# tier4/icp_rust

Measured on AMD Instinct MI355X. Metric: ICP iterations/sec on 1M-pt 3D pair, higher is better.
Workload: dtype f64

## Files before the change

### icp_rust_amd/_lib.py

```python
import ctypes as C
import os
import subprocess

_HERE = os.path.dirname(os.path.abspath(__file__))
_CSRC = os.path.join(_HERE, "csrc")
LIB_PATH = os.environ.get("ICP_MI355X_LIB") or os.path.join(_HERE, "lib", "libicp_mi355x.so")

OK, NONE, EMPTY_DST, NAN_INPUT, BAD_ARGUMENT, NO_DEVICE, HIP_ERROR, OUT_OF_MEMORY, RETRY_REPLICATED, RETRY_SHARDED = range(10)
NN_AUTO, NN_BRUTE, NN_GRID = 0, 1, 2


class Pose(C.Structure):

    _fields_ = [(n, C.c_double) for n in ("r00", "r10", "r01", "r11", "tx", "ty")]

    def as_tuple(self):
        return (self.r00, self.r10, self.r01, self.r11, self.tx, self.ty)


class BatchItem(C.Structure):

    _fields_ = [("src_first", C.c_uint64), ("n", C.c_uint64), ("dst_first", C.c_uint64), ("m", C.c_uint64),
                ("init", Pose)]

# ... 94 lines not shown
    "icp_estimate_transform_device": (C.c_int, [_vp, _vp, _vp, _sz, _pp, _vp]),
    "icp_nn_search_device": (C.c_int, [_vp, _vp, _sz, _vp]),
    "icp_weighted_gn_step_device": (C.c_int, [_vp, _vp, _vp, _sz, _pp, C.c_int, _dp, _dp]),
    "icp_shard_geometry": (C.c_int, [_sz, C.c_int, C.c_int, C.POINTER(C.c_int), C.POINTER(C.c_int),
                                     C.POINTER(C.c_int), C.POINTER(_sz)]),
    "icp_shard_histogram_words": (_sz, []),
    "icp_shard_candidates_bytes": (_sz, []),
    "icp_shard_partials_bytes": (_sz, [C.c_int]),
    "icp_shard_exchange_bytes": (_sz, [C.c_int]),
    "icp_shard_take_device": (C.c_int, [_vp, _vp, _vp, _sz, C.c_int, C.c_int, _sz]),
    "icp_shard_put_device": (C.c_int, [_vp, _vp, _vp, _sz, C.c_int, C.c_int, _sz]),
    "icp_shard_eval_hist_device": (C.c_int, [_vp, _vp, _vp, _sz, C.c_int, C.c_int, _pp, C.c_int, C.c_int,
                                             C.POINTER(_vp)]),
    "icp_shard_eval_compact_device": (C.c_int, [_vp, _vp]),
    "icp_shard_eval_finish_device": (C.c_int, [_vp, _vp, _dp, _dp]),
    "icp_create_multi": (C.c_int, [C.POINTER(_vp), C.c_int, _vp, _sz, C.POINTER(C.c_int), C.c_int]),
    "icp_multi_estimate": (C.c_int, [_vp, _vp, _sz, _pp, _sz, _pp, _vp, _vp]),
    "icp_multi_counters": (C.c_int, [_vp, C.POINTER(C.c_uint64)]),
    "icp_multi_loop_counters": (C.c_int, [_vp, C.POINTER(C.c_uint64)]),
    "icp_multi_pipe_iterations": (C.c_int, [_vp, C.POINTER(C.c_uint64)]),
    "icp_pipe_counters": (C.c_int, [_vp, C.POINTER(C.c_uint64)]),
    "icp_debug_sort_cells": (C.c_int, [_vp, _sz, C.c_uint, _vp, _vp]),
    "icp_set_fixed_point_exit": (C.c_int, [_vp, C.c_int]),
    "icp_shard_pipe_run_device": (C.c_int, [_vp, _vp, _sz, _sz, C.c_int, C.c_int, _pp, C.POINTER(_sz), _sz, _vp, _vp,
                                            C.POINTER(C.c_int)]),
    "icp_loop_inbox_bytes": (_sz, []),
    "icp_loop_inbox": (C.c_int, [_vp, C.c_int, C.POINTER(C.c_void_p)]),
    "icp_loop_inbox_ipc_handle": (C.c_int, [_vp, C.c_char_p]),
    "icp_loop_ipc_open": (C.c_int, [C.c_int, C.c_char_p, C.POINTER(C.c_void_p)]),
    "icp_loop_ipc_close": (C.c_int, [_vp]),
    "icp_loop_inbox_shm_name": (C.c_int, [_vp, C.c_char_p]),
    "icp_loop_inbox_shm_unlink": (C.c_int, [_vp]),
    "icp_loop_shm_open": (C.c_int, [C.c_int, C.c_char_p, C.POINTER(C.c_void_p)]),
    "icp_loop_shm_close": (C.c_int, [_vp]),
    "icp_loop_transport_probe": (C.c_int, [_vp, C.c_int, C.POINTER(C.c_int)]),
    "icp_reset_window_predictions": (C.c_int, [_vp]),
    "icp_shard_loop_connect": (C.c_int, [_vp, C.c_int, C.c_int, C.POINTER(C.c_void_p)]),
    "icp_shard_loop_launch_device": (C.c_int, [_vp, _vp, _vp, _sz, C.c_uint, C.c_uint, C.c_int, C.c_uint32, _pp, C.c_double,
                                               C.c_int, C.c_int]),
    "icp_shard_loop_wait": (C.c_int, [_vp, _pp, C.POINTER(C.c_double), _u32p, C.POINTER(C.c_int), C.POINTER(C.c_int), _u32p]),
    "icp_destroy_multi": (None, [_vp]),
    "icp_synchronize": (C.c_int, [_vp]),
    "icp_profile_enable": (C.c_int, [_vp, C.c_int]),
    "icp_profile_read": (C.c_int, [_vp, _dp, C.POINTER(C.c_uint64)]),
    "icp_reduce_geometry": (None, [_sz, C.POINTER(C.c_int), C.POINTER(C.c_int)]),
    "icp_nn_cert_counters": (C.c_int, [_vp, C.POINTER(C.c_uint64)]),
# ... 154 lines not shown
```

### icp_rust_amd/csrc/api.hip

```cpp
#include <dlfcn.h>
#include <fcntl.h>
#include <sys/mman.h>
#include <unistd.h>

#include <cfloat>
#include <chrono>
#include <cstdio>
#include <cstring>
#include <atomic>
#include <map>
#include <mutex>
#include <new>

#include "api_internal.hpp"

using namespace icp;
using namespace icp::api;

namespace icp {
namespace api {
int map_hip(hipError_t e) {
  switch (e) {
    case hipSuccess: return ICP_OK;
    case hipErrorOutOfMemory: return ICP_OUT_OF_MEMORY;
// ... 332 lines not shown
void free_handle(icp_handle *h) {
  (void)hipSetDevice(h->device);
  free_workspace(h->ws);
  (void)hipFree(h->d_dst_own);
  (void)hipFree(h->d_dst_soa);
  (void)hipFree(h->d_dst_f32);
  (void)hipFree(h->grid.d_start);
  (void)hipFree(h->grid.d_pts);
  (void)hipFree(h->grid.t_cell_of);
  (void)hipFree(h->grid.t_cnt);
  (void)hipFree(h->grid.t_btot);
  (void)hipFree(h->grid.t_part);
  (void)hipFree(h->grid.d_rcell);
  (void)hipFree(h->grid.d_rcell2);
  (void)hipFree(h->grid.d_start2);
  (void)hipFree(h->grid.d_pts2);
  (void)hipFree(h->grid.t_shift);
  (void)hipFree(h->grid.t_cell_new);
  (void)hipFree(h->grid.d_flag);
  (void)hipFree(h->qsort.d_cell_of);
  (void)hipFree(h->qsort.d_tmp);
  (void)hipFree(h->qsort.d_cert_lists);
  (void)hipFree(h->qsort.d_cert_ctr);
  (void)hipFree(h->qsort.d_perm);
  (void)hipFree(h->qsort.d_sorted);
  (void)hipFree(h->qsort.d_prev);
  (void)hipFree(h->shard.d_ordered);
  (void)hipFree(h->d_normals);
  (void)hipFree(h->d_dst_alt);
  (void)hipFree(h->d_normals_alt);
  (void)hipFree(h->d_plane_pairs);
  (void)hipFree(h->d_plane_fa);
  (void)hipFree(h->d_plane_fb);
  (void)hipFree(h->d_plane_stage);
  if (h->own_stream) (void)hipStreamDestroy(h->own_stream);
  delete h;
}

constexpr size_t kPoolMax = 2;
std::mutex g_pool_mu;
std::vector<icp_handle *> g_pool;

}

static void destroy_failed(icp_handle *h) {
  (void)hipSetDevice(h->device);
// ... 15 lines not shown

extern "C" void icp_destroy(icp_handle *h) {
  if (!h) return;
  (void)hipSetDevice(h->device);
  if (h->own_stream) (void)hipStreamSynchronize(h->own_stream);
  if (h->stream != h->own_stream) (void)hipStreamSynchronize(h->stream);
  if (h->ws.spec_stream) (void)hipStreamSynchronize(h->ws.spec_stream);
  for (auto *v : {&h->prof_events, &h->prof_free}) {
    for (auto &ev : *v) {
      (void)hipEventDestroy(ev.first);
      (void)hipEventDestroy(ev.second);
    }
    v->clear();
  }
  static const bool no_pool = getenv("ICP_NO_POOL") != nullptr;
  if (!no_pool) {
    Workspace &w = h->ws;
    h->m = 0;
    h->d_dst = nullptr;
    h->owns_dst = false;
    h->nn_mode = ICP_NN_AUTO;
    h->single_launch = true;
    h->fixed_point_exit = true;
    h->stream = h->own_stream;
    h->profile = 0;
    h->prof_seen = 0;
    h->grid.built = false;
    h->grid.appends_moved = h->grid.appends_rebuilt = 0;
    h->grid.crops_moved = h->grid.crops_rebuilt = 0;
    h->grid.thins_moved = h->grid.thins_rebuilt = 0;
    h->grid.filters_moved = h->grid.filters_rebuilt = 0;
    h->grid.removes_moved = h->grid.removes_rebuilt = 0;
    h->grid.queries_cell = h->grid.queries_caller = 0;
    h->grid.query_force = 0;
    h->qsort.valid = false;
    h->qsort.have_prev = false;
    h->qsort.slot_order = false;
    h->qsort.fold_n = 0;
    h->qsort.last_cert_ctr = nullptr;
    h->qsort.cert_searches = 0;
    h->qsort.have_certs = false;
    h->shard.active = false;
    h->shard.refined_ready = h->shard.attempt_refined = false;
    h->normals_m = 0;
    h->normals_k = 0;
    for (int k = 0; k < 5; ++k) {
// ... 45 lines not shown
static constexpr long kGridMinM = 8192;

int icp::api::resolved_nn_mode(const icp_handle *h) {
  if (h->nn_mode == ICP_NN_BRUTE || !h->grid.built) return ICP_NN_BRUTE;
  if (h->nn_mode == ICP_NN_GRID) return ICP_NN_GRID;
  return (long)h->m >= kGridMinM ? ICP_NN_GRID : ICP_NN_BRUTE;
}

static hipError_t launch_nn(icp_handle *h, const double *d_src, size_t n, const Pose *T, double *d_a,
                            double *d_b, uint32_t *d_idx) {
  Range range("icp: search (transform + exact nearest neighbour + pairs)");
  if (resolved_nn_mode(h) == ICP_NN_GRID) return launch_nn_grid(h, d_src, n, T, d_a, d_b, d_idx);
  return launch_nn_brute(h, d_src, n, T, d_a, d_b, d_idx);
}

extern "C" int icp_set_single_launch(icp_handle *h, int enable) {
  if (!h) return ICP_BAD_ARGUMENT;
  h->single_launch = enable != 0;
  return ICP_OK;
}
extern "C" int icp_set_fixed_point_exit(icp_handle *h, int enable) {
  if (!h) return ICP_BAD_ARGUMENT;
  h->fixed_point_exit = enable != 0;
  return ICP_OK;
}
extern "C" int icp_single_launch_counters(icp_handle *h, uint64_t out[3]) {
  if (!h || !out) return ICP_BAD_ARGUMENT;
  out[0] = h->ws.tiny_calls;
  out[1] = h->ws.tiny_evals;
  out[2] = h->ws.tiny_sorted;
  return ICP_OK;
}
extern "C" int icp_get_nn_mode(const icp_handle *h) {
  if (!h) return ICP_BAD_ARGUMENT;
  return resolved_nn_mode(h);
}
extern "C" int icp_set_stream(icp_handle *h, void *s) {
  if (!h) return ICP_BAD_ARGUMENT;
  h->stream = (hipStream_t)s;
  return ICP_OK;
}
extern "C" int icp_use_own_stream(icp_handle *h) {
  if (!h) return ICP_BAD_ARGUMENT;
  h->stream = h->own_stream;
  return ICP_OK;
}
// ... 880 lines not shown
```

### icp_rust_amd/csrc/common.hpp

```cpp
#pragma once
#include <hip/hip_runtime.h>

#include <cstddef>
#include <cstdint>
#include <cstdlib>
#include <utility>
#include <vector>

#include "pose.hpp"

namespace icp {


struct Range {
  explicit Range(const char *name);
  ~Range();
  Range(const Range &) = delete;
  Range &operator=(const Range &) = delete;
};

constexpr int kReduceThreads = 512;
constexpr int kReduceMaxBlocks = 256;
constexpr int kTreeMaxBlocks = 2048;
constexpr int kShardMaxWorld = 16;
// ... 257 lines not shown
struct QuerySort {
  bool valid = false;
  bool slot_order = false;
  bool identity = false;
  bool presorted = false;
  bool sort_only = false;
  size_t fold_n = 0;
  const double *src = nullptr;
  size_t n = 0, cap = 0;
  uint32_t *d_cell_of = nullptr;
  uint32_t *d_perm = nullptr;
  void *d_tmp = nullptr;
  size_t cap_tmp = 0;
  bool have_prev = false;
  PrevMatch *d_prev = nullptr;
  double *d_sorted = nullptr;
  bool have_certs = false, have_pose = false, have_pose_before = false;
  double decay_r = 0., decay_t = 0.;
  Pose last_pose;
  uint32_t *d_cert_lists = nullptr;
  unsigned *d_cert_ctr = nullptr, *last_cert_ctr = nullptr;
  unsigned cert_seq = 0;
  unsigned long long cert_searches = 0;
};

hipError_t stable_sort_cells(const uint32_t *keys_in, uint32_t *perm_out, unsigned n, unsigned bits, void *&tmp, size_t &cap_tmp,
                             hipStream_t s);

}

struct icp_handle {
  int dim = 0;
  size_t m = 0;
  int device = 0;
  int nn_mode = ICP_NN_AUTO;
  bool single_launch = true;
  bool fixed_point_exit = true;
  bool owns_dst = false;
  const double *d_dst = nullptr;
  double *d_dst_own = nullptr;
  size_t cap_dst_own = 0, cap_soa = 0, cap_f32 = 0;
  double *d_dst_soa = nullptr;
  float *d_dst_f32 = nullptr;
  size_t m_pad = 0;
  bool brute_valid = false;
  bool screen_valid = false;
  hipStream_t own_stream = nullptr;
  hipStream_t stream = nullptr;
  icp::Workspace ws;
  icp::Grid grid;
  icp::QuerySort qsort;
  struct ShardEval {
    icp::WinParams P;
    int kind = 2, rank = 0, world = 1, b0 = 0, b1 = 0, blocks = 0;
    size_t n_local = 0, n_total = 0;
    const double *d_a = nullptr;
    icp::Pose T;
    double *d_ordered = nullptr;
    bool active = false;
    icp::WinParams P2;
// ... 211 lines not shown
```

### icp_rust_amd/csrc/nn_grid.hip

```cpp
#include "common.hpp"
#include <type_traits>

namespace icp {

__device__ __forceinline__ int cell_coord(double v, double lo, double inv_h, int n) {
  double t = floor((v - lo) * inv_h);
  t = fmin(fmax(t, 0.), (double)(n - 1));
  return (int)t;
}

__global__ void k_grid_bbox(const double *__restrict__ dst, unsigned m, int dim, double *__restrict__ part) {
  __shared__ double smn[3][256], smx[3][256];
  double mn[3], mx[3];
  for (int d = 0; d < 3; ++d) {
    mn[d] = __builtin_huge_val();
    mx[d] = -__builtin_huge_val();
  }
  for (unsigned i = blockIdx.x * 256 + threadIdx.x; i < m; i += gridDim.x * 256)
    for (int d = 0; d < dim; ++d) {
      const double v = dst[(size_t)i * dim + d];
      mn[d] = fmin(mn[d], v);
      mx[d] = fmax(mx[d], v);
    }
  for (int d = 0; d < 3; ++d) {
// ... 929 lines not shown
                                                               GridParams g, const uint32_t *__restrict__ start,
                                                               const GridPoint *__restrict__ pts,
                                                               const double *__restrict__ dst, uint32_t *__restrict__ idx,
                                                               double2 *__restrict__ a, double2 *__restrict__ b,
                                                               PrevMatch *prev, CertDecay cd, unsigned xcd_chunk) {
  const unsigned k = xcd_wave(blockIdx.x, gridDim.x, xcd_chunk) * kGridThreads + threadIdx.x;
  if (k >= n) return;
  warm_query<DIM, CERT>(k, src, perm, T, g, start, pts, dst, idx, a, b, prev, cd);
}

#ifndef ICP_COOP_ITEMS
#define ICP_COOP_ITEMS 2
#endif
#ifndef ICP_COOP_ROWS
#define ICP_COOP_ROWS 4
#endif
#ifndef ICP_COOP_FLUSH_AT
#define ICP_COOP_FLUSH_AT 96
#endif
constexpr int kCoopItems = ICP_COOP_ITEMS;
constexpr int kCoopRows = ICP_COOP_ROWS;
constexpr int kCoopCandCap = 256;
constexpr int kCoopFlushAt = ICP_COOP_FLUSH_AT;
struct CoopLds {
  uint32_t pref[64];
  uint32_t rows_d[64][kCoopRows];
  uint32_t rows_o[64][kCoopRows];
  float4 oq[64];
  uint32_t obi[64];
  uint2 cand[kCoopCandCap];
  unsigned long long fkey[64];
  uint32_t fidx[64];
  uint32_t fwin[64];
};

#ifdef ICP_COOP_PROFILE
__device__ unsigned long long g_coop_prof[64][12];
__device__ long long g_coop_span[16384][2];
__device__ unsigned long long g_coop_rows[32];
#define COOP_STAMP(i)                                                  \
  do {                                                                 \
    asm volatile("s_waitcnt vmcnt(0) lgkmcnt(0)" ::: "memory");        \
    const long long now_ = wall_clock64();                             \
    cprof[i] += (unsigned long long)(now_ - ct_last);                  \
    ct_last = now_;                                                    \
  } while (0)
#define COOP_COUNT(i, v) (cprof[i] += (v))
#else
#define COOP_STAMP(i) ((void)0)
#define COOP_COUNT(i, v) ((void)0)
#endif

template <int DIM, bool SEEDED>
__device__ __forceinline__ void warm_wave(const unsigned k, const unsigned n, const double *__restrict__ src,
                                          const uint32_t *__restrict__ perm, Pose T, const GridParams &g,
                                          const uint32_t *__restrict__ start, const GridPoint *__restrict__ pts,
                                          const double *__restrict__ dst, uint32_t *__restrict__ idx,
                                          double2 *__restrict__ a, double2 *__restrict__ b, PrevMatch *prev, PrevMatch seed,
                                          CoopLds &S) {
  const unsigned lane = threadIdx.x;
#ifdef ICP_COOP_PROFILE
  unsigned long long cprof[12] = {0, 0, 0, 0, 0, 0, 0, 1, 0, 0, 0, 0};
  long long ct_last = wall_clock64();
  const long long ct_first = ct_last;
#endif
  const bool in_range = k < n;
  const unsigned kk = in_range ? k : n - 1;
  const unsigned i = perm ? perm[kk] : kk;
  double q[3];
  q[0] = src[(size_t)kk * DIM + 0];
  q[1] = src[(size_t)kk * DIM + 1];
  q[2] = DIM == 3 ? src[(size_t)kk * DIM + 2] : 0.;
  {
    const double nx = (T.r00 * q[0] + T.r01 * q[1]) + T.tx;
    const double ny = (T.r10 * q[0] + T.r11 * q[1]) + T.ty;
    q[0] = nx;
    q[1] = ny;
  }
  const PrevMatch pm = SEEDED ? seed : prev[kk];
  const bool no_match = pm.idx == 0xffffffffu;
  bool alive = in_range && !no_match;
  auto dist2 = [&](double tx, double ty, double tz) -> double {
// ... 165 lines not shown
    };
    ey(0);
    if (ny > 1) ey(1);
    if (ny > 2) {
      ey(2);
      ey(3);
    }
    ez(0);
    row(0);
    if (DIM == 3 && nz > 1) {
      ez(1);
      row(1);
      if (nz > 2) {
        ez(2);
        ez(3);
        row(2);
        row(3);
      }
    }
    if (on) mask = m;
  };
  make_mask(alive);
  const bool wave_tiles = __ballot(alive && (hi_c[1] - lo_c[1] >= 4 || hi_c[2] - lo_c[2] >= 4)) != 0ull;
#ifdef ICP_COOP_PROFILE
  unsigned rows_total = 0;
#endif
  for (;;) {
    int nr = 0;
    uint32_t rlo[kCoopRows], rhi[kCoopRows];
#pragma unroll
    for (int r = 0; r < kCoopRows; ++r) rlo[r] = rhi[r] = 0u;
    auto pick = [&](const bool on, uint32_t &d, uint32_t &o) -> bool {
      const bool take = on && mask != 0u;
      const int r = __ffs((int)mask) - 1;
      if (on) mask &= mask - 1u;
      const int jy = r & 3, jz = r >> 2;
      const uint32_t rb = ((uint32_t)(tz + jz) * g.n[1] + (uint32_t)(ty + jy)) * g.n[0];
      if (take) {
        d = rb + lo_c[0];
        o = rb + hi_c[0] + 1;
      }
      return take;
    };
#pragma unroll
    for (int r = 0; r < kCoopRows; ++r) {
      if (__ballot(mask != 0u) == 0ull) break;
      nr += pick(true, rlo[r], rhi[r]) ? 1 : 0;
    }
// ... 34 lines not shown
      sb[r] = start[rlo[r]];
      se[r] = start[rhi[r]];
    }
    uint32_t rd[kCoopRows], ro[kCoopRows], Q = 0;
#pragma unroll
    for (int r = 0; r < kCoopRows; ++r) {
      const uint32_t nq = ((nr > r) & (se[r] > sb[r])) ? ((se[r] - sb[r] + 3) >> 2) : 0u;
      ro[r] = Q;
      rd[r] = sb[r] - 4u * Q;
      Q += nq;
    }
    COOP_STAMP(2);
    uint32_t incl = Q;
#define ICP_SCAN_DPP(v, ctrl, rows) (uint32_t)__builtin_amdgcn_update_dpp(0, (int)(v), ctrl, rows, 0xf, true)
    incl += ICP_SCAN_DPP(incl, 0x111, 0xf);
    incl += ICP_SCAN_DPP(incl, 0x112, 0xf);
    incl += ICP_SCAN_DPP(incl, 0x114, 0xf);
    incl += ICP_SCAN_DPP(incl, 0x118, 0xf);
    incl += ICP_SCAN_DPP(incl, 0x142, 0xa);
    incl += ICP_SCAN_DPP(incl, 0x143, 0xc);
#undef ICP_SCAN_DPP
    const uint32_t total = (uint32_t)__builtin_amdgcn_readlane((int)incl, 63);
    S.pref[lane] = incl - Q;
#pragma unroll
    for (int r = 0; r < kCoopRows; ++r) {
      S.rows_d[lane][r] = rd[r];
      S.rows_o[lane][r] = ro[r];
    }
    __syncthreads();
    COOP_STAMP(3);
    auto batch = [&](auto ni_, const uint32_t w0) {
      constexpr int NI = decltype(ni_)::value;
      COOP_COUNT(9, 1);
      GridPoint t[4 * NI];
      unsigned own[NI];
      bool has[NI];
#pragma unroll
      for (int it = 0; it < NI; ++it) {
        const uint32_t w = w0 + 64u * it + lane;
        has[it] = w < total;
        const uint32_t wc = has[it] ? w : total - 1;
        unsigned L = 0;
#pragma unroll
        for (unsigned st = 32; st >= 1; st >>= 1)
          if (S.pref[L + st] <= wc) L += st;
        own[it] = L;
// ... 41 lines not shown
          cnt += (unsigned)__popcll(bal[u]);
        }
      }
    };
    {
      uint32_t w0 = 0;
      for (; w0 + 64u < total; w0 += 64u * kCoopItems) batch(std::integral_constant<int, kCoopItems>{}, w0);
      if (w0 < total) batch(std::integral_constant<int, 1>{}, w0);
    }
    __syncthreads();
    COOP_STAMP(4);
    if (cnt >= (unsigned)kCoopFlushAt) {
      flush();
      COOP_STAMP(5);
    }
  }
  COOP_STAMP(1);
  if (cnt > 0) flush();
  COOP_STAMP(5);
#ifdef ICP_COOP_PROFILE
  auto coop_report = [&]() {
    asm volatile("s_waitcnt vmcnt(0) lgkmcnt(0)" ::: "memory");
    cprof[6] += (unsigned long long)(wall_clock64() - ct_last);
    if (in_range) atomicAdd(&g_coop_rows[rows_total < 31u ? rows_total : 31u], 1ull);
    if (lane == 0) {
      for (int j = 0; j < 12; ++j) atomicAdd(&g_coop_prof[blockIdx.x & 63][j], cprof[j]);
      if (blockIdx.x < 16384u) {
        g_coop_span[blockIdx.x][0] = ct_first;
        g_coop_span[blockIdx.x][1] = wall_clock64();
      }
    }
  };
#endif

  auto emit = [&]() {
    if (!in_range) return;
    if (no_match) {
      if (SEEDED) prev[k] = pm;
      if (idx) idx[i] = 0;
      if (a) a[i] = make_double2(q[0], q[1]);
      if (b) b[i] = make_double2(dst[0], dst[1]);
      return;
    }
    if (bi == 0xffffffffu) {
      bi = 0;
      bx = dst[0];
      by = dst[1];
      bz = DIM == 3 ? dst[2] : 0.;
    }
    if (SEEDED || bi != pm.idx) {
      PrevMatch out;
      out.x = bx;
      out.y = by;
      out.z = bz;
      out.idx = bi;
      out.pad = 0;
      prev[k] = out;
    }
    if (idx) idx[i] = bi;
    if (a) a[i] = make_double2(q[0], q[1]);
    if (b) b[i] = make_double2(bx, by);
  };
  emit();
#ifdef ICP_COOP_PROFILE
  coop_report();
#endif
}

#ifdef ICP_COOP_WAVES
#define ICP_COOP_ATTR __attribute__((amdgpu_waves_per_eu(ICP_COOP_WAVES, ICP_COOP_WAVES)))
#else
#define ICP_COOP_ATTR
#endif
template <int DIM>
__global__ __launch_bounds__(kGridThreads) ICP_COOP_ATTR void k_nn_grid_warm_coop(const double *__restrict__ src,
                                                                    const uint32_t *__restrict__ perm, unsigned n, Pose T,
                                                                    GridParams g, const uint32_t *__restrict__ start,
                                                                    const GridPoint *__restrict__ pts,
                                                                    const double *__restrict__ dst, uint32_t *__restrict__ idx,
                                                                    double2 *__restrict__ a, double2 *__restrict__ b,
                                                                    PrevMatch *prev, unsigned xcd_chunk,
                                                                    const AheadPose *__restrict__ ahead) {
  __shared__ CoopLds S;
  if (ahead) {
    if (!ahead->valid) return;
    T = ahead->T;
  }
  const unsigned k = xcd_wave(blockIdx.x, gridDim.x, xcd_chunk) * kGridThreads + threadIdx.x;
  warm_wave<DIM, false>(k, n, src, perm, T, g, start, pts, dst, idx, a, b, prev, PrevMatch{0., 0., 0., 0xffffffffu, 0u}, S);
}

constexpr int kCertLists = 16;
constexpr int kCertCtrStride = 32;
constexpr int kCertThreads = 256;

template <int DIM>
__global__ __launch_bounds__(kCertThreads) void k_nn_cert(const double *__restrict__ src,
                                                          const uint32_t *__restrict__ perm, unsigned n, Pose T,
                                                          const double *__restrict__ dst, uint32_t *__restrict__ idx,
                                                          double2 *__restrict__ a, double2 *__restrict__ b,
                                                          const PrevMatch *__restrict__ prev, CertDecay cd,
                                                          uint32_t *__restrict__ lists, unsigned list_cap,
                                                          unsigned *ctr, unsigned *ctr_next) {
  __shared__ unsigned s_cnt[kCertThreads / 64], s_base;
  const unsigned k = blockIdx.x * kCertThreads + threadIdx.x;
  const int lane = threadIdx.x & 63, wave = threadIdx.x >> 6;
  if (blockIdx.x == 0 && threadIdx.x < kCertLists) ctr_next[threadIdx.x * kCertCtrStride] = 0;
  bool fail = false;
  if (k < n) {
    const unsigned i = perm ? perm[k] : k;
    double q[3];
    q[0] = src[(size_t)k * DIM + 0];
// ... 200 lines not shown
  if (n == 0) return hipSuccess;
  hipLaunchKernelGGL(k_unpermute_idx, dim3(((unsigned)n + 255) / 256), dim3(256), 0, h->stream, d_slot_idx,
                     (const uint32_t *)h->qsort.d_perm, (unsigned)n, d_out);
  return hipGetLastError();
}

hipError_t prepare_queries(icp_handle *h, const double *d_src, size_t n_, const Pose &T) {
  Grid &G = h->grid;
  QuerySort &Q = h->qsort;
  Q.valid = false;
  Q.fold_n = 0;
  if (!G.built || n_ == 0) return hipSuccess;
  const unsigned n = (unsigned)n_;
  hipError_t e;
  hipStream_t s = h->stream;
  if (n_ > Q.cap) {
    if ((e = hipStreamSynchronize(s)) != hipSuccess) return e;
    (void)hipFree(Q.d_cell_of);
    (void)hipFree(Q.d_perm);
    (void)hipFree(Q.d_sorted);
    (void)hipFree(Q.d_prev);
    (void)hipFree(Q.d_cert_lists);
    (void)hipFree(Q.d_cert_ctr);
    Q.last_cert_ctr = nullptr;
    Q.d_prev = nullptr;
    Q.d_cert_lists = nullptr;
    Q.d_cert_ctr = nullptr;
    Q.d_cell_of = Q.d_perm = nullptr;
    Q.d_sorted = nullptr;
    Q.cap = 0;
    Q.fold_n = 0;
    if ((e = hipMalloc(&Q.d_cell_of, n_ * 4)) != hipSuccess) return e;
    if ((e = hipMalloc(&Q.d_perm, n_ * 4)) != hipSuccess) return e;
    if ((e = hipMalloc(&Q.d_sorted, n_ * 3 * sizeof(double))) != hipSuccess) return e;
    if ((e = hipMalloc(&Q.d_prev, n_ * sizeof(PrevMatch))) != hipSuccess) return e;
    if ((e = hipMalloc(&Q.d_cert_lists, (n_ + (size_t)(kCertLists + 1) * kCertThreads) * sizeof(uint32_t))) != hipSuccess) return e;
    if ((e = hipMalloc(&Q.d_cert_ctr, (size_t)2 * kCertLists * kCertCtrStride * sizeof(unsigned))) != hipSuccess) return e;
    if ((e = hipMemsetAsync(Q.d_cert_ctr, 0, (size_t)2 * kCertLists * kCertCtrStride * sizeof(unsigned), s)) != hipSuccess) return e;
    Q.cert_seq = 0;
    Q.cap = n_;
  }
  Q.identity = (long)n <= kGridCoopMaxN || Q.presorted;
  Q.presorted = false;
  if (Q.identity) {
    Q.have_prev = false;
    Q.have_certs = false;
    Q.have_pose = Q.have_pose_before = false;
    Q.decay_r = Q.decay_t = 0.;
    Q.src = d_src;
    Q.n = n_;
    Q.valid = true;
    return hipSuccess;
  }
  const unsigned long long keys = (unsigned long long)G.p.n[2] * (unsigned long long)G.p.n[1] * (unsigned long long)G.p.n[0];
  hipLaunchKernelGGL(k_query_cell, dim3((n + 255) / 256), dim3(256), 0, s, d_src, n, h->dim, T, G.p, 0, Q.d_cell_of, 0);
  unsigned bits = 1;
  while (bits < 32 && (1ull << bits) < keys) ++bits;
  if ((e = stable_sort_cells(Q.d_cell_of, Q.d_perm, n, bits, Q.d_tmp, Q.cap_tmp, s)) != hipSuccess) return e;
  if (Q.sort_only) {
    Q.sort_only = false;
    Q.src = d_src;
    Q.n = n_;
    return hipGetLastError();
  }
  {
    const size_t pairs = ((size_t)n * h->dim + 1) / 2;
    hipLaunchKernelGGL(k_query_gather, dim3((unsigned)((pairs + 255) / 256)), dim3(256), 0, s, d_src, n, h->dim,
                       (const uint32_t *)Q.d_perm, Q.d_sorted);
  }
  Q.have_prev = false;
  Q.have_certs = false;
  Q.have_pose = Q.have_pose_before = false;
  Q.decay_r = Q.decay_t = 0.;
  if ((e = hipGetLastError()) != hipSuccess) return e;
  Q.src = d_src;
  Q.n = n_;
  Q.valid = true;
  return hipSuccess;
}

hipError_t launch_nn_grid_ahead(icp_handle *h, const double *d_src, size_t n_, const AheadPose *d_pose, double *d_a,
                                double *d_b, uint32_t *d_idx, bool *launched) {
  *launched = false;
  const Grid &G = h->grid;
  QuerySort &Q = h->qsort;
  if (n_ == 0 || n_ >= 0xffffffffull || !d_pose || h->m == 0 || !G.built || !G.p.f32_ok) return hipSuccess;
  const unsigned n = (unsigned)n_;
  if (!(Q.valid && Q.src == d_src && Q.n == n_ && Q.have_prev)) return hipSuccess;
  const bool coop = (long)n <= kGridCoopMaxN;
  const double *q_src = !Q.identity ? Q.d_sorted : d_src;
  const uint32_t *q_perm = (!Q.slot_order && !Q.identity) ? Q.d_perm : nullptr;
  hipEvent_t ev0 = nullptr, ev1 = nullptr;
  if (h->profile > 0 && (h->prof_seen++ % (unsigned)h->profile) == 0) {
    if (!h->prof_free.empty()) {
      ev0 = h->prof_free.back().first;
      ev1 = h->prof_free.back().second;
      h->prof_free.pop_back();
      (void)hipEventRecord(ev0, h->stream);
    } else if (hipEventCreate(&ev0) == hipSuccess && hipEventCreate(&ev1) == hipSuccess)
      (void)hipEventRecord(ev0, h->stream);
  }
  const unsigned blocks = (unsigned)(((size_t)n * (coop ? 4 : 1) + kGridThreads - 1) / kGridThreads);
  Q.have_pose = false;
  Q.have_certs = false;
  if (coop) {
    if (h->dim == 3)
      hipLaunchKernelGGL((k_nn_grid<3, true, false, 4>), dim3(blocks), dim3(kGridThreads), 0, h->stream, q_src, q_perm, n,
                         transform_identity(), G.p, G.d_start, G.d_pts, h->d_dst, d_idx, (double2 *)d_a, (double2 *)d_b,
                         (const PrevMatch *)Q.d_prev, Q.d_prev, d_pose);
    else
      hipLaunchKernelGGL((k_nn_grid<2, true, false, 4>), dim3(blocks), dim3(kGridThreads), 0, h->stream, q_src, q_perm, n,
                         transform_identity(), G.p, G.d_start, G.d_pts, h->d_dst, d_idx, (double2 *)d_a, (double2 *)d_b,
                         (const PrevMatch *)Q.d_prev, Q.d_prev, d_pose);
  } else if (h->dim == 3)
    hipLaunchKernelGGL(k_nn_grid_warm_coop<3>, dim3(blocks), dim3(kGridThreads), 0, h->stream, q_src, q_perm, n,
                       transform_identity(), G.p, G.d_start, G.d_pts, h->d_dst, d_idx, (double2 *)d_a, (double2 *)d_b, Q.d_prev,
                       (unsigned)kXcdChunk, d_pose);
  else
    hipLaunchKernelGGL(k_nn_grid_warm_coop<2>, dim3(blocks), dim3(kGridThreads), 0, h->stream, q_src, q_perm, n,
                       transform_identity(), G.p, G.d_start, G.d_pts, h->d_dst, d_idx, (double2 *)d_a, (double2 *)d_b, Q.d_prev,
                       (unsigned)kXcdChunk, d_pose);
  const hipError_t e = hipGetLastError();
  if (ev0 && ev1) {
    (void)hipEventRecord(ev1, h->stream);
    h->prof_events.emplace_back(ev0, ev1);
  }
  *launched = e == hipSuccess;
  return e;
}

hipError_t launch_nn_grid(icp_handle *h, const double *d_src, size_t n_, const Pose *Tp, double *d_a,
                          double *d_b, uint32_t *d_idx) {
  if (n_ == 0) return hipSuccess;
  const unsigned n = (unsigned)n_;
  const bool xform = Tp != nullptr;
  const Pose T = xform ? *Tp : transform_identity();
  const Grid &G = h->grid;
  const QuerySort &Q = h->qsort;
  const bool sorted = xform && Q.valid && Q.src == d_src && Q.n == n_;
  const double *q_src = (sorted && !Q.identity) ? Q.d_sorted : d_src;
  const uint32_t *q_perm = (sorted && !Q.slot_order && !Q.identity) ? Q.d_perm : nullptr;
  PrevMatch *q_prev_out = sorted ? Q.d_prev : nullptr;
  const PrevMatch *q_prev = (sorted && Q.have_prev) ? Q.d_prev : nullptr;
  if (sorted) h->qsort.have_prev = true;
// ... 63 lines not shown
        hipLaunchKernelGGL(k_nn_cert<2>, dim3(cblocks), dim3(kCertThreads), 0, h->stream, q_src, q_perm, n, T, h->d_dst,
                           d_idx, (double2 *)d_a, (double2 *)d_b, (const PrevMatch *)Q.d_prev, cd, QW.d_cert_lists,
                           list_cap, ctr, ctr_next);
        hipLaunchKernelGGL(k_nn_walk_lists<2>, wgrid, dim3(kGridThreads), 0, h->stream, q_src, q_perm, T, G.p, G.d_start,
                           G.d_pts, h->d_dst, d_idx, (double2 *)d_a, (double2 *)d_b, Q.d_prev, cd,
                           (const uint32_t *)QW.d_cert_lists, list_cap, (const unsigned *)ctr);
      }
    } else if (certs) {
      QW.have_certs = true;
      if (h->dim == 3)
        hipLaunchKernelGGL((k_nn_grid_warm<3, true>), dim3(blocks), dim3(kGridThreads), 0, h->stream, q_src, q_perm, n, T,
                           G.p, G.d_start, G.d_pts, h->d_dst, d_idx, (double2 *)d_a, (double2 *)d_b, Q.d_prev, cd, kXcdChunk);
      else
        hipLaunchKernelGGL((k_nn_grid_warm<2, true>), dim3(blocks), dim3(kGridThreads), 0, h->stream, q_src, q_perm, n, T,
                           G.p, G.d_start, G.d_pts, h->d_dst, d_idx, (double2 *)d_a, (double2 *)d_b, Q.d_prev, cd, kXcdChunk);
    } else if (seeded) {
      if (h->dim == 3)
        hipLaunchKernelGGL(k_nn_grid_seeded<3>, dim3(blocks), dim3(kGridThreads), 0, h->stream, q_src, q_perm, n, T, G.p,
                           G.d_start, G.d_pts, h->d_dst, d_idx, (double2 *)d_a, (double2 *)d_b, Q.d_prev);
      else
        hipLaunchKernelGGL(k_nn_grid_seeded<2>, dim3(blocks), dim3(kGridThreads), 0, h->stream, q_src, q_perm, n, T, G.p,
                           G.d_start, G.d_pts, h->d_dst, d_idx, (double2 *)d_a, (double2 *)d_b, Q.d_prev);
    } else {
      if (h->dim == 3)
        hipLaunchKernelGGL(k_nn_grid_warm_coop<3>, dim3(blocks), dim3(kGridThreads), 0, h->stream, q_src, q_perm, n, T,
                           G.p, G.d_start, G.d_pts, h->d_dst, d_idx, (double2 *)d_a, (double2 *)d_b, Q.d_prev, kXcdChunk,
                           (const AheadPose *)nullptr);
      else
        hipLaunchKernelGGL(k_nn_grid_warm_coop<2>, dim3(blocks), dim3(kGridThreads), 0, h->stream, q_src, q_perm, n, T,
                           G.p, G.d_start, G.d_pts, h->d_dst, d_idx, (double2 *)d_a, (double2 *)d_b, Q.d_prev, kXcdChunk,
                           (const AheadPose *)nullptr);
    }
    hipError_t we = hipGetLastError();
    if (ev0 && ev1) {
      (void)hipEventRecord(ev1, h->stream);
      h->prof_events.emplace_back(ev0, ev1);
    }
    return we;
  }
#define GRID(DIM, XF)                       \
  do {                                      \
    if (q_prev) {                           \
      GRID2(DIM, XF, false);                \
    } else {                                \
      GRID2(DIM, XF, true);                 \
    }                                       \
  } while (0)
#define GRID2(DIM, XF, CD)                  \
  do {                                      \
    if (coop) {                             \
      GRID3(DIM, XF, CD, 4);                \
    } else {                                \
      GRID3(DIM, XF, CD, 1);                \
    }                                       \
// ... 10 lines not shown
#undef GRID
#undef GRID2
#undef GRID3
  hipError_t e = hipGetLastError();
  if (ev0 && ev1) {
    (void)hipEventRecord(ev1, h->stream);
    h->prof_events.emplace_back(ev0, ev1);
  }
  return e;
}

#ifdef ICP_COOP_PROFILE
extern "C" int icp_debug_coop_rows(unsigned long long out[32], int reset) {
  if (hipMemcpyFromSymbol(out, HIP_SYMBOL(g_coop_rows), 32 * sizeof(unsigned long long)) != hipSuccess) return 1;
  if (reset) {
    unsigned long long z[32] = {0};
    if (hipMemcpyToSymbol(HIP_SYMBOL(g_coop_rows), z, sizeof(z)) != hipSuccess) return 1;
  }
  return 0;
}
extern "C" int icp_debug_coop_spans(long long *out, int n) {
  return hipMemcpyFromSymbol(out, HIP_SYMBOL(g_coop_span), (size_t)n * 2 * sizeof(long long)) == hipSuccess ? 0 : 1;
}
extern "C" int icp_debug_coop_profile(unsigned long long out[12], int reset) {
  unsigned long long all[64][12];
  if (hipMemcpyFromSymbol(all, HIP_SYMBOL(g_coop_prof), sizeof(all)) != hipSuccess) return 1;
  for (int j = 0; j < 12; ++j) {
    out[j] = 0;
    for (int i = 0; i < 64; ++i) out[j] += all[i][j];
  }
  if (reset) {
    memset(all, 0, sizeof(all));
    if (hipMemcpyToSymbol(HIP_SYMBOL(g_coop_prof), all, sizeof(all)) != hipSuccess) return 1;
  }
  return 0;
}
#endif

}
```

### include/icp_mi355x_debug.h

```cpp
#ifndef ICP_MI355X_DEBUG_H
#define ICP_MI355X_DEBUG_H

#include "icp_mi355x.h"

#ifdef __cplusplus
extern "C" {
#endif

int icp_gn_path_counters(icp_handle *h, uint64_t out[6]);

int icp_gn_loop_counters(icp_handle *h, uint64_t out[3]);
int icp_gn_loop_timeouts(icp_handle *h, uint64_t *out);
int icp_fixed_point_skips(icp_handle *h, uint64_t *out);

int icp_run_ahead_counters(icp_handle *h, uint64_t out[2]);

int icp_gn_filed_counters(icp_handle *h, uint64_t out[2]);

int icp_nn_cert_counters(icp_handle *h, uint64_t out[2]);

int icp_single_launch_counters(icp_handle *h, uint64_t out[3]);

int icp_grid_append_counters(const icp_handle *h, uint64_t out[2]);

int icp_grid_crop_counters(const icp_handle *h, uint64_t out[2]);

int icp_grid_thin_counters(const icp_handle *h, uint64_t out[2]);
int icp_grid_outlier_counters(const icp_handle *h, uint64_t out[2]);

int icp_multi_counters(const icp_multi *M, uint64_t out[2]);

int icp_multi_loop_counters(const icp_multi *M, uint64_t out[3]);

int icp_multi_pipe_iterations(const icp_multi *M, uint64_t *out);
int icp_pipe_counters(icp_handle *h, uint64_t out[4]);

int icp_set_fixed_point_exit(icp_handle *h, int enable);

int icp_debug_sort_cells(const uint32_t *keys, size_t n, unsigned bits, uint32_t *keys_out, uint32_t *perm_out);

int icp_batch_counters(icp_batch *b, uint64_t out[4]);
int icp_batch_evaluate_counters(icp_batch *b, uint64_t out[3]);
int icp_batch_line_counters(icp_batch *b, uint64_t out[4]);
int icp_batch_line_quality_counters(icp_batch *b, uint64_t out[4]);
int icp_batch_line_gated_counters(icp_batch *b, uint64_t out[4]);
int icp_batch_plane_counters(icp_batch *b, uint64_t out[4]);
int icp_debug_plane_batch_plan(unsigned threads, unsigned m, uint32_t out[4]);
int icp_batch_plane_gated_counters(icp_batch *b, uint64_t out[4]);
int icp_debug_plane_gated_batch_plan(unsigned threads, unsigned m, uint32_t out[4]);
int icp_batch_plane_quality_counters(icp_batch *b, uint64_t out[4]);
int icp_debug_plane_quality_batch_plan(unsigned m, uint32_t out[4]);
int icp_batch_gated_counters(icp_batch *b, uint64_t out[4]);
int icp_grid_remove_counters(const icp_handle *h, uint64_t out[2]);
int icp_query_counters(const icp_handle *h, uint64_t out[2]);
int icp_query_force_order(icp_handle *h, int mode);

int icp_profile_enable(icp_handle *h, int enable);
int icp_profile_read(icp_handle *h, double *nn_kernel_ms, uint64_t *nn_kernel_launches);

#ifdef __cplusplus
}
// ... 4 lines not shown
```

Before: 10320.

## Schedule warm coop search chunks longest-first using measured per-chunk cost

```diff
diff --git a/icp_rust_amd/_lib.py b/icp_rust_amd/_lib.py
--- a/icp_rust_amd/_lib.py
+++ b/icp_rust_amd/_lib.py
@@ -140,6 +140,8 @@
     "icp_pipe_counters": (C.c_int, [_vp, C.POINTER(C.c_uint64)]),
     "icp_debug_sort_cells": (C.c_int, [_vp, _sz, C.c_uint, _vp, _vp]),
     "icp_set_fixed_point_exit": (C.c_int, [_vp, C.c_int]),
+    "icp_set_search_order": (C.c_int, [_vp, C.c_int]),
+    "icp_search_order_table": (C.c_int, [_vp, _u32p, _sz, C.POINTER(_sz)]),
     "icp_shard_pipe_run_device": (C.c_int, [_vp, _vp, _sz, _sz, C.c_int, C.c_int, _pp, C.POINTER(_sz), _sz, _vp, _vp,
                                             C.POINTER(C.c_int)]),
     "icp_loop_inbox_bytes": (_sz, []),
diff --git a/icp_rust_amd/csrc/api.hip b/icp_rust_amd/csrc/api.hip
--- a/icp_rust_amd/csrc/api.hip
+++ b/icp_rust_amd/csrc/api.hip
@@ -378,6 +378,8 @@
   (void)hipFree(h->qsort.d_tmp);
   (void)hipFree(h->qsort.d_cert_lists);
   (void)hipFree(h->qsort.d_cert_ctr);
+  (void)hipFree(h->qsort.d_chunk_cost);
+  (void)hipFree(h->qsort.d_chunk_order);
   (void)hipFree(h->qsort.d_perm);
   (void)hipFree(h->qsort.d_sorted);
   (void)hipFree(h->qsort.d_prev);
@@ -439,6 +441,7 @@
     h->nn_mode = ICP_NN_AUTO;
     h->single_launch = true;
     h->fixed_point_exit = true;
+    h->search_order = true;
     h->stream = h->own_stream;
     h->profile = 0;
     h->prof_seen = 0;
@@ -530,6 +533,20 @@
 extern "C" int icp_set_fixed_point_exit(icp_handle *h, int enable) {
   if (!h) return ICP_BAD_ARGUMENT;
   h->fixed_point_exit = enable != 0;
+  return ICP_OK;
+}
+extern "C" int icp_set_search_order(icp_handle *h, int enable) {
+  if (!h) return ICP_BAD_ARGUMENT;
+  h->search_order = enable != 0;
+  return ICP_OK;
+}
+extern "C" int icp_search_order_table(icp_handle *h, uint32_t *out, size_t cap, size_t *chunks) {
+  if (!h || !chunks || (cap > 0 && !out)) return ICP_BAD_ARGUMENT;
+  HIP_TRY(hipSetDevice(h->device));
+  HIP_TRY(hipStreamSynchronize(h->stream));
+  *chunks = h->qsort.d_chunk_order ? h->qsort.order_chunks : 0;
+  const size_t k = *chunks < cap ? *chunks : cap;
+  if (k > 0) HIP_TRY(hipMemcpy(out, h->qsort.d_chunk_order, k * sizeof(uint32_t), hipMemcpyDeviceToHost));
   return ICP_OK;
 }
 extern "C" int icp_single_launch_counters(icp_handle *h, uint64_t out[3]) {
diff --git a/icp_rust_amd/csrc/common.hpp b/icp_rust_amd/csrc/common.hpp
--- a/icp_rust_amd/csrc/common.hpp
+++ b/icp_rust_amd/csrc/common.hpp
@@ -303,6 +303,10 @@
   unsigned *d_cert_ctr = nullptr, *last_cert_ctr = nullptr;
   unsigned cert_seq = 0;
   unsigned long long cert_searches = 0;
+  unsigned *d_chunk_cost = nullptr;
+  uint32_t *d_chunk_order = nullptr;
+  bool have_order = false;
+  size_t order_chunks = 0;
 };
 
 hipError_t stable_sort_cells(const uint32_t *keys_in, uint32_t *perm_out, unsigned n, unsigned bits, void *&tmp, size_t &cap_tmp,
@@ -317,6 +321,7 @@
   int nn_mode = ICP_NN_AUTO;
   bool single_launch = true;
   bool fixed_point_exit = true;
+  bool search_order = true;
   bool owns_dst = false;
   const double *d_dst = nullptr;
   double *d_dst_own = nullptr;
diff --git a/icp_rust_amd/csrc/nn_grid.hip b/icp_rust_amd/csrc/nn_grid.hip
--- a/icp_rust_amd/csrc/nn_grid.hip
+++ b/icp_rust_amd/csrc/nn_grid.hip
@@ -975,6 +975,9 @@
 constexpr int kCoopRows = ICP_COOP_ROWS;
 constexpr int kCoopCandCap = 256;
 constexpr int kCoopFlushAt = ICP_COOP_FLUSH_AT;
+constexpr unsigned kCostPerRound = 200;
+constexpr int kOrderClasses = 128;
+
 struct CoopLds {
   uint32_t pref[64];
   uint32_t rows_d[64][kCoopRows];
@@ -990,7 +993,11 @@
 #ifdef ICP_COOP_PROFILE
 __device__ unsigned long long g_coop_prof[64][12];
 __device__ long long g_coop_span[16384][2];
+__device__ unsigned g_coop_work[16384][4];
 __device__ unsigned long long g_coop_rows[32];
+#ifdef ICP_COOP_SPANS_ONLY
+#define COOP_STAMP(i) ((void)0)
+#else
 #define COOP_STAMP(i)                                                  \
   do {                                                                 \
     asm volatile("s_waitcnt vmcnt(0) lgkmcnt(0)" ::: "memory");        \
@@ -998,6 +1005,7 @@
     cprof[i] += (unsigned long long)(now_ - ct_last);                  \
     ct_last = now_;                                                    \
   } while (0)
+#endif
 #define COOP_COUNT(i, v) (cprof[i] += (v))
 #else
 #define COOP_STAMP(i) ((void)0)
@@ -1010,7 +1018,7 @@
                                           const uint32_t *__restrict__ start, const GridPoint *__restrict__ pts,
                                           const double *__restrict__ dst, uint32_t *__restrict__ idx,
                                           double2 *__restrict__ a, double2 *__restrict__ b, PrevMatch *prev, PrevMatch seed,
-                                          CoopLds &S) {
+                                          CoopLds &S, unsigned *cost_slot = nullptr) {
   const unsigned lane = threadIdx.x;
 #ifdef ICP_COOP_PROFILE
   unsigned long long cprof[12] = {0, 0, 0, 0, 0, 0, 0, 1, 0, 0, 0, 0};
@@ -1222,8 +1230,9 @@
   };
   make_mask(alive);
   const bool wave_tiles = __ballot(alive && (hi_c[1] - lo_c[1] >= 4 || hi_c[2] - lo_c[2] >= 4)) != 0ull;
+  unsigned cost = 0;
 #ifdef ICP_COOP_PROFILE
-  unsigned rows_total = 0;
+  unsigned rows_total = 0, quads_total = 0;
 #endif
   for (;;) {
     int nr = 0;
@@ -1304,6 +1313,10 @@
 #undef ICP_SCAN_DPP
     const uint32_t total = (uint32_t)__builtin_amdgcn_readlane((int)incl, 63);
     S.pref[lane] = incl - Q;
+    if (!SEEDED) cost += total + kCostPerRound;
+#ifdef ICP_COOP_PROFILE
+    quads_total += total;
+#endif
 #pragma unroll
     for (int r = 0; r < kCoopRows; ++r) {
       S.rows_d[lane][r] = rd[r];
@@ -1391,12 +1404,26 @@
   auto coop_report = [&]() {
     asm volatile("s_waitcnt vmcnt(0) lgkmcnt(0)" ::: "memory");
     cprof[6] += (unsigned long long)(wall_clock64() - ct_last);
+#ifndef ICP_COOP_SPANS_ONLY
     if (in_range) atomicAdd(&g_coop_rows[rows_total < 31u ? rows_total : 31u], 1ull);
+#endif
+    unsigned rows_sum = rows_total, rows_max = rows_total;
+    for (int st = 1; st < 64; st <<= 1) {
+      const unsigned o = (unsigned)__shfl_xor((int)rows_sum, st), m = (unsigned)__shfl_xor((int)rows_max, st);
+      rows_sum += o;
+      rows_max = m > rows_max ? m : rows_max;
+    }
     if (lane == 0) {
+#ifndef ICP_COOP_SPANS_ONLY
       for (int j = 0; j < 12; ++j) atomicAdd(&g_coop_prof[blockIdx.x & 63][j], cprof[j]);
+#endif
       if (blockIdx.x < 16384u) {
         g_coop_span[blockIdx.x][0] = ct_first;
         g_coop_span[blockIdx.x][1] = wall_clock64();
+        g_coop_work[blockIdx.x][0] = quads_total;
+        g_coop_work[blockIdx.x][1] = (unsigned)cprof[8];
+        g_coop_work[blockIdx.x][2] = rows_sum;
+        g_coop_work[blockIdx.x][3] = rows_max;
       }
     }
   };
@@ -1431,6 +1458,7 @@
     if (b) b[i] = make_double2(bx, by);
   };
   emit();
+  if (!SEEDED && cost_slot && lane == 0) atomicAdd(cost_slot, cost);
 #ifdef ICP_COOP_PROFILE
   coop_report();
 #endif
@@ -1449,14 +1477,57 @@
                                                                     const double *__restrict__ dst, uint32_t *__restrict__ idx,
                                                                     double2 *__restrict__ a, double2 *__restrict__ b,
                                                                     PrevMatch *prev, unsigned xcd_chunk,
-                                                                    const AheadPose *__restrict__ ahead) {
+                                                                    const AheadPose *__restrict__ ahead,
+                                                                    const uint32_t *__restrict__ chunk_order,
+                                                                    unsigned *chunk_cost) {
   __shared__ CoopLds S;
   if (ahead) {
     if (!ahead->valid) return;
     T = ahead->T;
   }
-  const unsigned k = xcd_wave(blockIdx.x, gridDim.x, xcd_chunk) * kGridThreads + threadIdx.x;
-  warm_wave<DIM, false>(k, n, src, perm, T, g, start, pts, dst, idx, a, b, prev, PrevMatch{0., 0., 0., 0xffffffffu, 0u}, S);
+  unsigned w = xcd_wave(blockIdx.x, gridDim.x, xcd_chunk);
+  if (chunk_order && xcd_chunk) w = chunk_order[w / xcd_chunk] * xcd_chunk + w % xcd_chunk;
+  const unsigned k = w * kGridThreads + threadIdx.x;
+  warm_wave<DIM, false>(k, n, src, perm, T, g, start, pts, dst, idx, a, b, prev, PrevMatch{0., 0., 0., 0xffffffffu, 0u}, S,
+                        (chunk_cost && xcd_chunk) ? chunk_cost + w / xcd_chunk : nullptr);
+}
+
+__global__ __launch_bounds__(64) void k_chunk_order(const unsigned *__restrict__ cost, unsigned nfull, unsigned nch,
+                                                    uint32_t *__restrict__ order) {
+  __shared__ unsigned s_cnt[kOrderClasses][64];
+  const unsigned lane = threadIdx.x;
+  const unsigned per = (nfull + 63u) / 64u;
+  const unsigned c0 = lane * per < nfull ? lane * per : nfull, c1 = c0 + per < nfull ? c0 + per : nfull;
+  unsigned mx = 0;
+  for (unsigned c = c0; c < c1; ++c) mx = cost[c] > mx ? cost[c] : mx;
+  for (int st = 1; st < 64; st <<= 1) {
+    const unsigned o = (unsigned)__shfl_xor((int)mx, st);
+    mx = o > mx ? o : mx;
+  }
+  auto cls = [&](unsigned v) -> unsigned {
+    return (unsigned)(kOrderClasses - 1) - (unsigned)(((unsigned long long)v * kOrderClasses) / ((unsigned long long)mx + 1ull));
+  };
+  for (int j = 0; j < kOrderClasses; ++j) s_cnt[j][lane] = 0u;
+  for (unsigned c = c0; c < c1; ++c) ++s_cnt[cls(cost[c])][lane];
+  __syncthreads();
+  unsigned *flat = &s_cnt[0][0];
+  constexpr unsigned kRun = (unsigned)kOrderClasses * 64u / 64u;
+  unsigned sum = 0;
+  for (unsigned j = 0; j < kRun; ++j) sum += flat[lane * kRun + j];
+  unsigned incl = sum;
+  for (int st = 1; st < 64; st <<= 1) {
+    const unsigned o = (unsigned)__shfl_up((int)incl, st);
+    if (lane >= (unsigned)st) incl += o;
+  }
+  unsigned run = incl - sum;
+  for (unsigned j = 0; j < kRun; ++j) {
+    const unsigned v = flat[lane * kRun + j];
+    flat[lane * kRun + j] = run;
+    run += v;
+  }
+  __syncthreads();
+  for (unsigned c = c0; c < c1; ++c) order[s_cnt[cls(cost[c])][lane]++] = c;
+  for (unsigned c = nfull + lane; c < nch; c += 64u) order[c] = c;
 }
 
 constexpr int kCertLists = 16;
@@ -1703,6 +1774,10 @@
     (void)hipFree(Q.d_prev);
     (void)hipFree(Q.d_cert_lists);
     (void)hipFree(Q.d_cert_ctr);
+    (void)hipFree(Q.d_chunk_cost);
+    (void)hipFree(Q.d_chunk_order);
+    Q.d_chunk_cost = nullptr;
+    Q.d_chunk_order = nullptr;
     Q.last_cert_ctr = nullptr;
     Q.d_prev = nullptr;
     Q.d_cert_lists = nullptr;
@@ -1719,8 +1794,13 @@
     if ((e = hipMalloc(&Q.d_cert_ctr, (size_t)2 * kCertLists * kCertCtrStride * sizeof(unsigned))) != hipSuccess) return e;
     if ((e = hipMemsetAsync(Q.d_cert_ctr, 0, (size_t)2 * kCertLists * kCertCtrStride * sizeof(unsigned), s)) != hipSuccess) return e;
     Q.cert_seq = 0;
+    const size_t chunks = ((n_ + kGridThreads - 1) / kGridThreads + kXcdChunk - 1) / kXcdChunk;
+    if ((e = hipMalloc(&Q.d_chunk_cost, chunks * sizeof(unsigned))) != hipSuccess) return e;
+    if ((e = hipMalloc(&Q.d_chunk_order, chunks * sizeof(uint32_t))) != hipSuccess) return e;
     Q.cap = n_;
   }
+  Q.have_order = false;
+  Q.order_chunks = 0;
   Q.identity = (long)n <= kGridCoopMaxN || Q.presorted;
   Q.presorted = false;
   if (Q.identity) {
@@ -1754,6 +1834,7 @@
   Q.have_pose = Q.have_pose_before = false;
   Q.decay_r = Q.decay_t = 0.;
   if ((e = hipGetLastError()) != hipSuccess) return e;
+
   Q.src = d_src;
   Q.n = n_;
   Q.valid = true;
@@ -1782,6 +1863,7 @@
       (void)hipEventRecord(ev0, h->stream);
   }
   const unsigned blocks = (unsigned)(((size_t)n * (coop ? 4 : 1) + kGridThreads - 1) / kGridThreads);
+  const uint32_t *order = (h->search_order && Q.slot_order && Q.have_order) ? Q.d_chunk_order : nullptr;
   Q.have_pose = false;
   Q.have_certs = false;
   if (coop) {
@@ -1796,11 +1878,11 @@
   } else if (h->dim == 3)
     hipLaunchKernelGGL(k_nn_grid_warm_coop<3>, dim3(blocks), dim3(kGridThreads), 0, h->stream, q_src, q_perm, n,
                        transform_identity(), G.p, G.d_start, G.d_pts, h->d_dst, d_idx, (double2 *)d_a, (double2 *)d_b, Q.d_prev,
-                       (unsigned)kXcdChunk, d_pose);
+                       (unsigned)kXcdChunk, d_pose, order, (unsigned *)nullptr);
   else
     hipLaunchKernelGGL(k_nn_grid_warm_coop<2>, dim3(blocks), dim3(kGridThreads), 0, h->stream, q_src, q_perm, n,
                        transform_identity(), G.p, G.d_start, G.d_pts, h->d_dst, d_idx, (double2 *)d_a, (double2 *)d_b, Q.d_prev,
-                       (unsigned)kXcdChunk, d_pose);
+                       (unsigned)kXcdChunk, d_pose, order, (unsigned *)nullptr);
   const hipError_t e = hipGetLastError();
   if (ev0 && ev1) {
     (void)hipEventRecord(ev1, h->stream);
@@ -1910,14 +1992,28 @@
         hipLaunchKernelGGL(k_nn_grid_seeded<2>, dim3(blocks), dim3(kGridThreads), 0, h->stream, q_src, q_perm, n, T, G.p,
                            G.d_start, G.d_pts, h->d_dst, d_idx, (double2 *)d_a, (double2 *)d_b, Q.d_prev);
     } else {
+      const bool ordered = h->search_order && Q.slot_order && QW.d_chunk_cost && QW.d_chunk_order;
+      const uint32_t *order = (ordered && QW.have_order) ? QW.d_chunk_order : nullptr;
+      unsigned *cost = (ordered && !QW.have_order) ? QW.d_chunk_cost : nullptr;
+      const unsigned nch = (blocks + kXcdChunk - 1) / kXcdChunk;
+      if (cost) {
+        const hipError_t ze = hipMemsetAsync(cost, 0, (size_t)nch * sizeof(unsigned), h->stream);
+        if (ze != hipSuccess) return ze;
+      }
       if (h->dim == 3)
         hipLaunchKernelGGL(k_nn_grid_warm_coop<3>, dim3(blocks), dim3(kGridThreads), 0, h->stream, q_src, q_perm, n, T,
                            G.p, G.d_start, G.d_pts, h->d_dst, d_idx, (double2 *)d_a, (double2 *)d_b, Q.d_prev, kXcdChunk,
-                           (const AheadPose *)nullptr);
+                           (const AheadPose *)nullptr, order, cost);
       else
         hipLaunchKernelGGL(k_nn_grid_warm_coop<2>, dim3(blocks), dim3(kGridThreads), 0, h->stream, q_src, q_perm, n, T,
                            G.p, G.d_start, G.d_pts, h->d_dst, d_idx, (double2 *)d_a, (double2 *)d_b, Q.d_prev, kXcdChunk,
-                           (const AheadPose *)nullptr);
+                           (const AheadPose *)nullptr, order, cost);
+      if (cost) {
+        const unsigned nfull = blocks / (8u * kXcdChunk) * 8u;
+        hipLaunchKernelGGL(k_chunk_order, dim3(1), dim3(64), 0, h->stream, (const unsigned *)cost, nfull, nch, QW.d_chunk_order);
+        QW.have_order = true;
+        QW.order_chunks = nch;
+      }
     }
     hipError_t we = hipGetLastError();
     if (ev0 && ev1) {
@@ -1974,6 +2070,9 @@
 extern "C" int icp_debug_coop_spans(long long *out, int n) {
   return hipMemcpyFromSymbol(out, HIP_SYMBOL(g_coop_span), (size_t)n * 2 * sizeof(long long)) == hipSuccess ? 0 : 1;
 }
+extern "C" int icp_debug_coop_work(unsigned *out, int n) {
+  return hipMemcpyFromSymbol(out, HIP_SYMBOL(g_coop_work), (size_t)n * 4 * sizeof(unsigned)) == hipSuccess ? 0 : 1;
+}
 extern "C" int icp_debug_coop_profile(unsigned long long out[12], int reset) {
   unsigned long long all[64][12];
   if (hipMemcpyFromSymbol(all, HIP_SYMBOL(g_coop_prof), sizeof(all)) != hipSuccess) return 1;
diff --git a/include/icp_mi355x_debug.h b/include/icp_mi355x_debug.h
--- a/include/icp_mi355x_debug.h
+++ b/include/icp_mi355x_debug.h
@@ -37,6 +37,9 @@
 
 int icp_set_fixed_point_exit(icp_handle *h, int enable);
 
+int icp_set_search_order(icp_handle *h, int enable);
+int icp_search_order_table(icp_handle *h, uint32_t *out, size_t cap, size_t *chunks);
+
 int icp_debug_sort_cells(const uint32_t *keys, size_t n, unsigned bits, uint32_t *keys_out, uint32_t *perm_out);
 
 int icp_batch_counters(icp_batch *b, uint64_t out[4]);
diff --git a/profiles/search_tail.py b/profiles/search_tail.py
--- /dev/null
+++ b/profiles/search_tail.py
@@ -0,0 +1,129 @@
+import ctypes as C, os, sys
+ROOT = os.path.dirname(os.path.dirname(os.path.abspath(__file__))); sys.path.insert(0, ROOT)
+import numpy as np
+
+SIMDS = 256 * 4
+TICK_US = 0.01
+CHUNK = 16
+
+
+def xcd_wave(block, nblocks, chunk=CHUNK):
+    per = 8 * chunk
+    full = nblocks // per * per
+    sc, r = block // per, block % per
+    return np.where(block >= full, block, sc * per + (r & 7) * chunk + (r >> 3))
+
+
+def ranks(v):
+    order = np.argsort(v, kind="stable")
+    r = np.empty(len(v)); r[order] = np.arange(len(v))
+    _, inv, cnt = np.unique(v, return_inverse=True, return_counts=True)
+    s = np.zeros(len(cnt)); np.add.at(s, inv, r)
+    return (s / cnt)[inv]
+
+
+def spearman(x, y):
+    rx, ry = ranks(x), ranks(y)
+    return float(np.corrcoef(rx, ry)[0, 1])
+
+
+def report(name, sp, wk, out=sys.stdout):
+    sp = sp - sp[:, 0].min()
+    life = (sp[:, 1] - sp[:, 0]) * TICK_US
+    end = sp[:, 1].max() * TICK_US
+    nb = len(sp)
+    p = lambda *a: print(*a, file=out)
+    p(f"== {name}: {nb} waves, first start to last end {end:.2f} us")
+    p(f"wave lifetime us: mean {life.mean():.2f} median {np.median(life):.2f} p90 {np.percentile(life, 90):.2f} "
+      f"p99 {np.percentile(life, 99):.2f} max {life.max():.2f}")
+    p("occupancy (waves resident at t, per SIMD chip-wide; waves started / retired in [t, t + 1 us)):")
+    t_under = None
+    peak_seen = False
+    for t in np.arange(0.0, end, 1.0):
+        tt = t / TICK_US
+        res = int(np.sum((sp[:, 0] <= tt) & (sp[:, 1] > tt)))
+        st = int(np.sum((sp[:, 0] >= tt) & (sp[:, 0] < tt + 100)))
+        rt = int(np.sum((sp[:, 1] >= tt) & (sp[:, 1] < tt + 100)))
+        p(f"  t = {t:5.1f} us: {res:5d} waves ({res / SIMDS:.2f} per SIMD), started {st:5d}, retired {rt:5d}")
+    grid = np.arange(0.0, end, 0.1)
+    resid = np.array([np.sum((sp[:, 0] <= t / TICK_US) & (sp[:, 1] > t / TICK_US)) for t in grid])
+    full = np.nonzero(resid >= 4 * SIMDS)[0]
+    if len(full):
+        t_under = grid[full[-1]] + 0.1
+        p(f"under-filled end: fewer than 4 waves per SIMD from t = {t_under:.1f} us to the end at {end:.2f} us: {end - t_under:.2f} us")
+        t_head = grid[full[0]]
+        p(f"head: 4 waves per SIMD first reached at t = {t_head:.1f} us")
+    else:
+        p(f"the launch never holds 4 waves per SIMD chip-wide (peak {resid.max() / SIMDS:.2f})")
+    last_start = sp[:, 0].max() * TICK_US
+    p(f"last wave starts at {last_start:.2f} us; waves retiring after it: {int(np.sum(sp[:, 1] * TICK_US > last_start))}")
+    q, rnd, rows, rmax = (wk[:, j].astype(np.float64) for j in range(4))
+    p("rank correlation of a wave's lifetime with its work counts:")
+    for nm, v in (("quads in its lists", q), ("rounds of rows", rnd), ("rows summed over lanes", rows), ("rows of its fullest lane", rmax),
+                  ("quads + 64 * rounds", q + 64 * rnd), ("quads + 128 * rounds", q + 128 * rnd), ("quads + 256 * rounds", q + 256 * rnd)):
+        p(f"  {nm:28s} {spearman(life, v):+.3f}")
+    A = np.stack([np.ones(nb), q, rnd], 1)
+    coef, *_ = np.linalg.lstsq(A, life, rcond=None)
+    fit = A @ coef
+    p(f"least squares: lifetime us = {coef[0]:.2f} + {coef[1]:.4f} * quads + {coef[2]:.2f} * rounds; "
+      f"R^2 {1 - np.sum((life - fit) ** 2) / np.sum((life - life.mean()) ** 2):.3f}")
+    p(f"work counts per wave: quads mean {q.mean():.0f} p90 {np.percentile(q, 90):.0f} max {q.max():.0f}; rounds mean {rnd.mean():.2f} max {rnd.max():.0f}")
+    wave = xcd_wave(np.arange(nb), nb)
+    ch = wave // CHUNK
+    nch = ch.max() + 1
+    c_life = np.zeros(nch); np.add.at(c_life, ch, life)
+    c_q = np.zeros(nch); np.add.at(c_q, ch, q)
+    c_r = np.zeros(nch); np.add.at(c_r, ch, rnd)
+    c_end = np.zeros(nch); np.maximum.at(c_end, ch, sp[:, 1] * TICK_US)
+    c_start = np.full(nch, 1e30); np.minimum.at(c_start, ch, sp[:, 0] * TICK_US)
+    p(f"chunks of {CHUNK} waves: {nch}; summed lifetime per chunk us: median {np.median(c_life):.0f} p90 {np.percentile(c_life, 90):.0f} max {c_life.max():.0f}")
+    p(f"  rank correlation of a chunk's summed lifetime with its quads {spearman(c_life, c_q):+.3f}, rounds {spearman(c_life, c_r):+.3f}, "
+      f"quads + 128 * rounds {spearman(c_life, c_q + 128 * c_r):+.3f}")
+    late = np.argsort(-c_end)[:12]
+    p("  the chunks that retire last: (chunk, first start us, last end us, summed lifetime / median)")
+    p("   " + ", ".join(f"({c}, {c_start[c]:.1f}, {c_end[c]:.1f}, {c_life[c] / np.median(c_life):.2f})" for c in late))
+    started_late = c_start > np.percentile(c_start, 75)
+    p(f"  chunks that start in the last quarter: summed lifetime / median: mean {np.mean(c_life[started_late]) / np.median(c_life):.2f}, "
+      f"max {np.max(c_life[started_late]) / np.median(c_life):.2f}")
+    return end - t_under if t_under is not None else None
+
+
+def main():
+    if len(sys.argv) > 2 and sys.argv[1] == "--report":
+        d = sys.argv[2]
+        for f in sorted(os.listdir(d)):
+            if f.startswith("spans_") and f.endswith(".npy"):
+                tag = f[len("spans_"):-4]
+                report(tag, np.load(os.path.join(d, f)), np.load(os.path.join(d, "work_" + tag + ".npy")))
+        return
+    out_dir = sys.argv[1] if len(sys.argv) > 1 else None
+    import torch
+    import icp_rust_amd as I
+    from icp_rust_amd import synth
+    n = m = 1_000_000
+    src, dst = synth.synthetic_pair(n, m)
+    d_src, d_dst = torch.from_numpy(src).cuda(), torch.from_numpy(dst).cuda()
+    icp = I.Icp3d(d_dst)
+    L = C.CDLL(os.environ["ICP_MI355X_LIB"])
+    L.icp_debug_coop_spans.argtypes = [C.c_void_p, C.c_int]
+    L.icp_debug_coop_work.argtypes = [C.c_void_p, C.c_int]
+    nb = (n + 63) // 64
+    for _ in range(5):
+        icp.estimate(d_src, I.Transform(), 20)
+    for k, rep in ((20, 0), (20, 1), (20, 2), (2, 0), (3, 0), (10, 0)):
+        icp.estimate(d_src, I.Transform(), k)
+        torch.cuda.synchronize()
+        sp = np.zeros((nb, 2), dtype=np.int64)
+        wk = np.zeros((nb, 4), dtype=np.uint32)
+        assert L.icp_debug_coop_spans(sp.ctypes.data, nb) == 0 and L.icp_debug_coop_work(wk.ctypes.data, nb) == 0
+        tag = f"iter{k:02d}_{rep}"
+        if out_dir:
+            os.makedirs(out_dir, exist_ok=True)
+            np.save(os.path.join(out_dir, f"spans_{tag}.npy"), sp)
+            np.save(os.path.join(out_dir, f"work_{tag}.npy"), wk)
+        report(f"search {k} of estimate(src, I, {k}), sample {rep}", sp, wk)
+    icp.close()
+
+
+if __name__ == "__main__":
+    main()
```

Result: no change. 10440 (median of 6 runs) (+1.2%).
